# cristianpjensen/thesis-pai-reconstruction

Hardware: NVIDIA B200
Metric: pix2pix_gan_train_images_per_sec_256x256 (higher is better)
Workload: dtype bf16

## Files before the change

### include/pai_b200.h

```cpp
#ifndef PAI_B200_H
#define PAI_B200_H

#ifdef __cplusplus
extern "C" {
#endif

#define PAI_ACT_NONE 0
#define PAI_ACT_LEAKY 1
#define PAI_ACT_RELU 2
#define PAI_ACT_TANH 3

#define PAI_DTYPE_F32 0
#define PAI_DTYPE_BF16 1

const char* pai_last_error(void);
int pai_version(void);
int pai_reserve_sms(int n);

int pai_conv4x4_fprop(const void* x, int n, int h, int w, int cin, int x_ld, const void* w_packed, int cout,
                      int cout_pad, int stride, const float* bias, int act, float slope, void* y, int y_ld,
                      int y_f32, int n_tile, float* splitk_ws, void* stream);

int pai_conv4x4_fprop_dual(const void* x, int n, int h, int w, int cin, int x_ld, const void* w_packed, int cout,
                           int cout_pad, int stride, const float* bias, int act, float slope, void* y, int y_ld, void* y2,
                           int y2_ld, int act2, int n_tile, void* stream);

int pai_convT4x4s2_fprop(const void* x, int n, int h, int w, int cin, int x_ld, const void* w_packed, int cout,
                         int cout_pad, const float* bias, int act, float slope, void* y, int y_ld, int y_f32,
                         int n_tile, float* splitk_ws, void* stream);
int pai_conv4x4_fprop_bnstats(const void* x, int n, int h, int w, int cin, int x_ld, const void* w_packed, int cout,
                              int cout_pad, int stride, const float* bias, void* y, int y_ld, int n_tile,
                              float* bn_partials, int bn_rows, void* stream);
int pai_convT4x4s2_fprop_bnstats(const void* x, int n, int h, int w, int cin, int x_ld, const void* w_packed, int cout,
                                 int cout_pad, const float* bias, void* y, int y_ld, int n_tile, float* bn_partials,
                                 int bn_rows, void* stream);
int pai_conv4x4_dgrad_act(const void* gy, int n, int h, int w, int cout, int gy_ld, const void* w_packed_dgrad, int cin,
                          int cin_pad, const void* saved_act, float slope, void* gx, int gx_ld, int n_tile,
                          float* colsum_partials, int rows, void* stream);

int pai_conv4x4_wgrad(const void* x, int n, int h, int w, int cin, int x_ld, const void* gy, int cout, int gy_ld,
                      int stride, float* dw, int splitk, void* stream);
int pai_convT4x4s2_wgrad(const void* x, int n, int h, int w, int cin, int x_ld, const void* gy, int cout, int gy_ld,
                         float* dw, int splitk, void* stream);

int pai_ssim_psnr_fwd(const void* pred, const void* target, int dtype, int n, int h, int w, int denormalize,
                      float* ssim_sum, float* band_sum, float* sse, float* full_map, void* stream);
int pai_ssim_psnr_bwd(const void* pred, const void* target, int dtype, int n, int h, int w, int denormalize,
                      const float* g_ssim_sum, const float* g_sse, void* workspace, void* grad_pred, void* stream);
long long pai_ssim_bwd_workspace_bytes(int n, int h, int w);

int pai_bn_stats(const void* x, long long m, int c, int ld, float* sums, void* stream);
int pai_bn_finalize(const float* sums, long long m, int c, const float* gamma, const float* beta, float eps,
                    float momentum, int training, float* running_mean, float* running_var, float* scale_shift,
                    void* stream);
int pai_bn_finalize_partials(const float* sums, int nparts, long long m, int c, const float* gamma, const float* beta,
                             float eps, float momentum, int training, float* running_mean, float* running_var,
                             float* scale_shift, void* stream);
int pai_bn_apply_act(const void* x, long long m, int c, int ld, const float* scale_shift, void* out1, int ld1,
                     int act1, void* out2, int ld2, int act2, float slope, void* stream);
int pai_bn_bwd_reduce(const void* x, long long m, int c, int ld, const float* scale_shift, const void* g1, int ldg1,
                      int act1, const void* g2, int ldg2, int act2, float slope, float* sums, void* stream);
int pai_bn_bwd_apply(const void* x, long long m, int c, int ld, const float* scale_shift, const void* g1, int ldg1,
                     int act1, const void* g2, int ldg2, int act2, float slope, const float* sums,
                     const float* gamma, void* dx, int lddx, void* stream);
int pai_act_bwd(const void* x, long long m, int c, int ld, const void* g1, int ldg1, int act1, const void* g2, int ldg2,
                int act2, float slope, float* sums2c, void* dx, int lddx, void* stream);
// ... 129 lines not shown
```

### thesis-pai-reconstruction_b200/csrc/igemm.cu

```cuda
#include <stdio.h>
#include <stdlib.h>

#include "pai_common.cuh"
#include "pai_epilogue.cuh"
#include "pai_kernels.h"

namespace pai {

#ifdef PAI_PROFILE_ROLES
#define ROLE_T0() const long long _t0 = clock64()
#define ROLE_ADD(var) var += clock64() - _t0
#else
#define ROLE_T0()
#define ROLE_ADD(var)
#endif

static constexpr int kThreads = 256;
static constexpr int kFpropThreads = 384;
static constexpr int kMaxStages = 8;

struct __align__(8) PipeSmem {
    uint64_t full[kMaxStages];
    uint64_t empty[kMaxStages];
    uint64_t acc_full[2];
    uint64_t acc_empty[2];
    uint64_t mask_full[8];
    uint32_t tmem_base;
};

template <bool PAIR, bool MASKED>
__global__ void __launch_bounds__(kFpropThreads, 1)
igemm_fprop_kernel(const __grid_constant__ CUtensorMap tm_a, const __grid_constant__ CUtensorMap tm_b,
                   const __grid_constant__ IgemmOutMaps om, const IgemmFpropParams p) {
    pdl_launch_dependents();
    extern __shared__ uint8_t smem_raw[];
    __shared__ PipeSmem ps;
    __shared__ __align__(1024) uint4 stage_buf[8][32 * 8];
    uint8_t* smem = reinterpret_cast<uint8_t*>((reinterpret_cast<uintptr_t>(smem_raw) + 1023) & ~uintptr_t(1023));

    const int warp = threadIdx.x >> 5, lane = threadIdx.x & 31;
    const int n_tile = p.n_tile;
    const bool fused = p.fused_phases != 0;
    const uint32_t rank = PAIR ? cluster_ctarank() : 0u;
    const int cta_n = PAIR ? n_tile / 2 : n_tile;
    const uint32_t a_bytes = 128 * 128;
    const uint32_t b_bytes = (uint32_t)cta_n * 128;
    const int ksub = p.ksub;
    const uint32_t sub_bytes = a_bytes + (fused ? 4 : 1) * b_bytes;
    const uint32_t stage_bytes = (uint32_t)ksub * sub_bytes;
    const int stages = p.stages;
    const int num_kb = (fused ? 9 : p.ntaps) * p.kc_per_tap;
    const int acc_n = fused ? 4 * n_tile : n_tile;
    const uint32_t acc_cols = tmem_cols_for(acc_n);
    const int total_tiles = p.n_tiles * p.m_tiles * p.phases * p.splitk;
    const int worker = PAIR ? (int)(blockIdx.x >> 1) : (int)blockIdx.x;
    const int workers = PAIR ? (int)(gridDim.x >> 1) : (int)gridDim.x;

// ... 8 lines not shown
        }
        for (int a = 0; a < 2; ++a) {
            mbar_init(&ps.acc_full[a], 1);
            mbar_init(&ps.acc_empty[a], PAIR ? 16 : 8);
        }
        if (MASKED)
            for (int w = 0; w < 8; ++w) mbar_init(&ps.mask_full[w], 1);
        mbar_fence_init();
    }
    if (warp == 2) {
        if (PAIR)
            tmem_alloc_pair(&ps.tmem_base, 2 * acc_cols);
        else
            tmem_alloc(&ps.tmem_base, 2 * acc_cols);
    }
    tc_fence_before();
    if (PAIR)
        cluster_sync_all();
    else
        __syncthreads();
    tc_fence_after();
    const uint32_t tmem_base = ps.tmem_base;
    pdl_wait();

    long long prof_wait = 0, prof_wait2 = 0, prof_total = 0, prof_fence = 0, prof_issue = 0, prof_commit = 0;
    (void)prof_wait, (void)prof_wait2, (void)prof_total, (void)prof_fence, (void)prof_issue, (void)prof_commit;
    const int pidx = warp == 0 ? 0 : (warp == 2 ? 1 : (warp == 3 ? 2 : -1));
    if (pidx >= 0) {
        if (elect_one()) {
            constexpr int P = 3;
            int g = 0, mine = pidx;
            int stage = pidx;
            uint32_t phase = 0;
            while (stage >= stages) stage -= stages, phase ^= 1;
            const int brow = PAIR ? (int)rank * cta_n : 0;
#ifdef PAI_PROFILE_ROLES
            const long long tstart = clock64();
#endif
            for (int t = worker; t < total_tiles; t += workers) {
                int ks, tt, nt, r, mt, phase_idx, tw, th, tn;
                p.fd_splitk.divmod(t, tt, ks);
                p.fd_n_tiles.divmod(tt, r, nt);
                p.fd_m_tiles.divmod(r, phase_idx, mt);
                if (PAIR) mt = 2 * mt + (int)rank;
                p.fd_tiles_w.divmod(mt, mt, tw);
                p.fd_tiles_h.divmod(mt, tn, th);
// ... 398 lines not shown
                        } else {
#pragma unroll
                            for (int j = 0; j < 16; ++j)
                                if (col0 + cc + j < p.cout) o[j] = apply_act(f[j], p.act, p.slope);
                        }
                    } else {
                        store_bf16_16(reinterpret_cast<__nv_bfloat16*>(p.out) + off + cc, f, p.act, p.slope,
                                      vec_ok && col0 + cc + 16 <= p.cout, p.cout - (col0 + cc));
                    }
                    if (p.out2 != nullptr)
                        store_bf16_16(reinterpret_cast<__nv_bfloat16*>(p.out2) + off2 + cc, f, p.act2, p.slope,
                                      vec_ok && col0 + cc + 16 <= p.cout, p.cout - (col0 + cc));
                }
            }
            if (!released) release_acc();
#ifdef PAI_PROFILE_ROLES
            prof_total += clock64() - twork;
#endif
        }
        if (p.bn_part != nullptr) flush_stats();
        if (lane == 0) bulk_wait_group0();
#ifdef PAI_PROFILE_ROLES
        if (blockIdx.x == 0 && threadIdx.x == 128)
            printf("[roles] epilogue warp 4: waiting for a full accumulator %lld cyc, working %lld cyc over %d tiles\n", prof_wait, prof_total, it);
#endif
    }
    tc_fence_before();
    if (PAIR)
        cluster_sync_all();
    else
        __syncthreads();
    if (warp == 2) {
        tc_fence_after();
        if (PAIR)
            tmem_dealloc_pair(tmem_base, 2 * acc_cols);
        else
            tmem_dealloc(tmem_base, 2 * acc_cols);
    }
}

__global__ void __launch_bounds__(kThreads, 1)
igemm_wgrad_kernel(const __grid_constant__ CUtensorMap tm_u, const __grid_constant__ CUtensorMap tm_s,
                   const IgemmWgradParams p) {
    pdl_launch_dependents();
    extern __shared__ uint8_t smem_raw[];
    __shared__ PipeSmem ps;
    uint8_t* smem = reinterpret_cast<uint8_t*>((reinterpret_cast<uintptr_t>(smem_raw) + 1023) & ~uintptr_t(1023));

    const int warp = threadIdx.x >> 5, lane = threadIdx.x & 31;
    const int mb = p.mb, nbt = p.nbt;
    const uint32_t blk_bytes = 64 * 128;
    const uint32_t a_bytes = 2 * mb * blk_bytes;
    const uint32_t stage_bytes = a_bytes + nbt * blk_bytes;
    const int stages = p.stages;
    const int n_cols = nbt * 64;
    const uint32_t tmem_cols = tmem_cols_for(mb * 256);

    const long long units = (long long)p.tiles * p.kblocks;
    const long long u_begin = units * blockIdx.x / gridDim.x, u_end = units * (blockIdx.x + 1) / gridDim.x;

// ... 20 lines not shown
    const int pidx = warp == 0 ? 0 : (warp == 2 ? 1 : (warp == 3 ? 2 : -1));
    if (pidx >= 0) {
        if (elect_one()) {
            constexpr int P = 3;
            int stage = pidx;
            uint32_t phase = 0;
            while (stage >= stages) stage -= stages, phase ^= 1;
            for (long long u = u_begin + pidx; u < u_end; u += P) {
                const int tile = (int)(u / p.kblocks);
                int mt = (int)(u - (long long)tile * p.kblocks);
                const int ng = tile % p.n_groups, cu0 = (tile / p.n_groups) * 128 * mb;
                const int tw = mt % p.tiles_w;
                mt /= p.tiles_w;
                const int th = mt % p.tiles_h;
                const int tn = mt / p.tiles_h;
                const int w0 = tw * p.bw, h0 = th * p.bh, n0 = tn * p.bn;
                mbar_wait(&ps.empty[stage], phase ^ 1);
                uint8_t* sa = smem + (size_t)stage * stage_bytes;
                uint8_t* sb = sa + a_bytes;
                mbar_expect_tx(&ps.full[stage], stage_bytes);
                for (int i = 0; i < 2 * mb; ++i)
                    tma_load_5d(sa + i * blk_bytes, &tm_u, &ps.full[stage], cu0 + i * 64, w0, 0, h0, n0);
                for (int nb = 0; nb < nbt; ++nb) {
                    const int blk = ng * nbt + nb, tap = blk / p.cs_blocks, cb = blk - tap * p.cs_blocks;
                    tma_load_5d(sb + nb * blk_bytes, &tm_s, &ps.full[stage], p.tap_c[tap] + cb * 64, w0 + p.tap_w[tap],
                                p.tap_p[tap], h0 + p.tap_h[tap], n0);
                }
                stage += P;
                while (stage >= stages) stage -= stages, phase ^= 1;
            }
        }
    } else if (warp == 1) {
        if (elect_one()) {
            const uint32_t idesc = umma_idesc_bf16(128, n_cols, 1, 1);
            int stage = 0;
            uint32_t phase = 0;
            int seg = 0;
            long long u = u_begin;
            while (u < u_end) {
                const long long tile_end = (u / p.kblocks + 1) * p.kblocks;
                const long long seg_end = tile_end < u_end ? tile_end : u_end;
                mbar_wait(&ps.acc_empty[0], (seg & 1) ^ 1);
                tc_fence_after();
                bool first = true;
                for (; u < seg_end; ++u) {
                    mbar_wait(&ps.full[stage], phase);
                    tc_fence_after();
// ... 14 lines not shown
                        stage = 0;
                        phase ^= 1;
                    }
                }
                umma_commit(&ps.acc_full[0]);
                ++seg;
            }
        }
    } else if (warp >= 4) {
        const int q = warp & 3;
        const int r = q * 32 + lane;
        int seg = 0;
        long long u = u_begin;
        while (u < u_end) {
            const int tile = (int)(u / p.kblocks);
            const long long tile_end = (long long)(tile + 1) * p.kblocks;
            u = tile_end < u_end ? tile_end : u_end;
            const int ng = tile % p.n_groups, cu0 = (tile / p.n_groups) * 128 * mb;
            mbar_wait(&ps.acc_full[0], seg & 1);
            tc_fence_after();
            for (int a = 0; a < mb; ++a) {
                const int row = cu0 + a * 128 + r;
                const bool row_ok = row < p.cu;
                for (int nb = 0; nb < nbt; ++nb) {
                    const int blk = ng * nbt + nb, tap = blk / p.cs_blocks, cb = blk - tap * p.cs_blocks;
                    float* o = p.out + ((size_t)tap * p.cu + row) * (size_t)p.cs + cb * 64;
#pragma unroll
                    for (int c = 0; c < 64; c += 16) {
                        uint32_t v[16];
                        __syncwarp();
                        tmem_ld_16(tmem_base + ((uint32_t)(q * 32) << 16) + (uint32_t)(a * 256 + nb * 64 + c), v);
                        tmem_ld_wait();
                        if (row_ok) {
#pragma unroll
                            for (int j = 0; j < 16; j += 4)
                                red_add_v4(o + c + j, __uint_as_float(v[j]), __uint_as_float(v[j + 1]),
                                           __uint_as_float(v[j + 2]), __uint_as_float(v[j + 3]));
                        }
                    }
                }
            }
            tc_fence_before();
            __syncwarp();
            if (lane == 0) mbar_arrive_relaxed(&ps.acc_empty[0]);
            ++seg;
        }
    }
    tc_fence_before();
// ... 119 lines not shown
    if (sms < 0) return -1;
    if (blocks > sms * 8) blocks = sms * 8;
    PAI_CUDA_OK(launch_pdl(splitk_finish_kernel, dim3((unsigned)blocks), dim3(256), 0, stream, 1, ws, total, cout, bias, act, slope, y, y_ld, y_f32));
    PAI_CUDA_OK(cudaGetLastError());
    return 0;
}

int launch_igemm_wgrad(const CUtensorMap& tm_u, const CUtensorMap& tm_s, IgemmWgradParams p, cudaStream_t stream) {
    const size_t stage_bytes = (size_t)(2 * p.mb + p.nbt) * 8192;
    p.stages = pick_stages(stage_bytes, 196 * 1024);
    const size_t smem = stage_bytes * p.stages + 1024;
    static DeviceOnce once;
    const int dev = current_device(), num_sms = persistent_ctas(dev);
    if (num_sms < 0) return -1;
    if (once.need(dev)) {
        PAI_CUDA_OK(cudaFuncSetAttribute(igemm_wgrad_kernel, cudaFuncAttributeMaxDynamicSharedMemorySize, 200 * 1024));
        once.mark(dev);
    }
    const long long units = (long long)p.tiles * p.kblocks;
    long long grid = units / 4 > p.tiles ? units / 4 : p.tiles;
    if (grid > num_sms) grid = num_sms;
    if (grid < 1) grid = 1;
    if (p.max_ctas > 0 && grid > p.max_ctas) grid = p.max_ctas;
    PAI_CUDA_OK(launch_pdl(igemm_wgrad_kernel, dim3((unsigned)grid), dim3(kThreads), smem, stream, 1, tm_u, tm_s, p));
    PAI_CUDA_OK(cudaGetLastError());
    return 0;
}

}
```

### thesis-pai-reconstruction_b200/csrc/pai_api.cu

```cuda
#include <stdarg.h>
#include <stdio.h>
#include <stdlib.h>
#include <string.h>

#include <cudaTypedefs.h>

#include "pai_common.cuh"
#include "pai_kernels.h"

namespace pai {

static thread_local char g_err[512] = "";

void set_error(const char* fmt, ...) {
    va_list ap;
    va_start(ap, fmt);
    vsnprintf(g_err, sizeof(g_err), fmt, ap);
    va_end(ap);
}

int cuda_fail(cudaError_t e, const char* what) {
    set_error("CUDA error %d (%s) at %s", (int)e, cudaGetErrorString(e), what);
    return -1;
}
// ... 387 lines not shown
                         int cout_pad, const float* bias, int act, float slope, void* y, int y_ld, int y_f32,
                         int n_tile, float* splitk_ws, void* stream) {
    return convT4x4s2_fprop_impl(x, n, h, w, cin, x_ld, w_packed, cout, cout_pad, bias, act, slope, y, y_ld, y_f32, n_tile,
                                 splitk_ws, nullptr, 0, stream);
}
int pai_convT4x4s2_fprop_bnstats(const void* x, int n, int h, int w, int cin, int x_ld, const void* w_packed, int cout,
                                 int cout_pad, const float* bias, void* y, int y_ld, int n_tile, float* bn_partials,
                                 int bn_rows, void* stream) {
    PAI_REQUIRE(bn_partials != nullptr && bn_rows > 0, "pai_convT4x4s2_fprop_bnstats: null partial-sum buffer");
    return convT4x4s2_fprop_impl(x, n, h, w, cin, x_ld, w_packed, cout, cout_pad, bias, PAI_ACT_NONE, 0.f, y, y_ld, 0,
                                 n_tile, nullptr, bn_partials, bn_rows, stream);
}

int pai_conv4x4_dgrad_act(const void* gy, int n, int h, int w, int cout, int gy_ld, const void* w_packed_dgrad, int cin,
                          int cin_pad, const void* saved_act, float slope, void* gx, int gx_ld, int n_tile,
                          float* colsum_partials, int rows, void* stream) {
    PAI_REQUIRE(saved_act != nullptr, "pai_conv4x4_dgrad_act: null saved activation");
    PAI_REQUIRE(colsum_partials == nullptr || rows > 0, "pai_conv4x4_dgrad_act: bad partial-sum buffer");
    return convT4x4s2_fprop_impl(gy, n, h, w, cout, gy_ld, w_packed_dgrad, cin, cin_pad, nullptr, PAI_ACT_NONE, 0.f, gx,
                                 gx_ld, 0, n_tile, nullptr, colsum_partials, rows, stream, saved_act, slope);
}

static int wgrad_common(const void* u, int un, int uh, int uw, int cu, int u_ld, const void* s, int sh, int sw,
                        int cs, int s_ld, int stride, float* dw, int splitk, cudaStream_t stream, const char* who) {
    PAI_REQUIRE(u && s && dw, "%s: null pointer", who);
    PAI_REQUIRE(cu % 64 == 0 && cs % 64 == 0, "%s: channel counts (%d rows, %d cols) must be multiples of 64", who, cu,
                cs);
    PAI_REQUIRE(aligned16(u) && aligned16(s) && u_ld % 8 == 0 && s_ld % 8 == 0, "%s: operands must be 16 B aligned",
                who);
    PixBox b = pick_box(uw, uh, un, 64);
    CUtensorMap tm_u, tm_s;
    int rc = map_unit(&tm_u, u, un, uh, uw, cu, u_ld, b);
    if (rc) return rc;
    if (stride == 2) {
        PAI_REQUIRE(s_ld == cs && sh % 2 == 0 && sw % 2 == 0, "%s: the stride-2 operand must be dense with even h,w",
                    who);
        rc = map_split(&tm_s, s, un, sh, sw, cs, b);
    } else {
        rc = map_unit(&tm_s, s, un, sh, sw, cs, s_ld, b);
    }
    if (rc) return rc;
    IgemmWgradParams p;
    memset(&p, 0, sizeof(p));
    p.bw = b.bw, p.bh = b.bh, p.bn = b.bn, p.tiles_w = b.tiles_w, p.tiles_h = b.tiles_h, p.tiles_n = b.tiles_n;
    p.cu = cu, p.cs = cs, p.out = dw;
    for (int ky = 0; ky < 4; ++ky)
        for (int kx = 0; kx < 4; ++kx) {
            int t = ky * 4 + kx;
            if (stride == 2) {
                int qx, px, qy, py;
                s2_tap(kx, &qx, &px);
                s2_tap(ky, &qy, &py);
                p.tap_c[t] = px * cs, p.tap_w[t] = qx, p.tap_p[t] = py, p.tap_h[t] = qy;
            } else if (stride == 1) {
                p.tap_c[t] = 0, p.tap_w[t] = kx - 1, p.tap_p[t] = 0, p.tap_h[t] = ky - 1;
            }
        }
    if (stride == 3)
        for (int t = 0; t < 9; ++t) p.tap_c[t] = 0, p.tap_w[t] = t % 3 - 1, p.tap_p[t] = 0, p.tap_h[t] = t / 3 - 1;
    const int ntaps = stride == 0 ? 1 : (stride == 3 ? 9 : 16);
    p.kblocks = b.tiles_w * b.tiles_h * b.tiles_n;
    p.cs_blocks = cs / 64;
    const int nb_total = ntaps * p.cs_blocks;
    p.nbt = nb_total % 4 == 0 ? 4 : (nb_total % 2 == 0 ? 2 : 1);
    p.n_groups = nb_total / p.nbt;
    p.mb = cu > 128 ? 2 : 1;
    p.tiles = ((cu + 128 * p.mb - 1) / (128 * p.mb)) * p.n_groups;
    p.max_ctas = splitk > 0 ? splitk * p.tiles : 0;
    return launch_igemm_wgrad(tm_u, tm_s, p, stream);
}

int pai_conv4x4_wgrad(const void* x, int n, int h, int w, int cin, int x_ld, const void* gy, int cout, int gy_ld,
                      int stride, float* dw, int splitk, void* stream) {
    PAI_REQUIRE(stride == 1 || stride == 2, "pai_conv4x4_wgrad: stride must be 1 or 2");
    const int ho = stride == 2 ? h / 2 : h - 1, wo = stride == 2 ? w / 2 : w - 1;
    return wgrad_common(gy, n, ho, wo, cout, gy_ld, x, h, w, cin, x_ld, stride, dw, splitk, (cudaStream_t)stream,
                        "pai_conv4x4_wgrad");
}

int pai_pointwise_wgrad(const void* u, long long m, int cu, int u_ld, const void* s, int cs, int s_ld, float* dw,
                        int splitk, void* stream) {
    PAI_REQUIRE(m > 0 && m < (1LL << 31), "pai_pointwise_wgrad: bad row count");
    return wgrad_common(u, 1, 1, (int)m, cu, u_ld, s, 1, (int)m, cs, s_ld, 0, dw, splitk, (cudaStream_t)stream,
                        "pai_pointwise_wgrad");
}

int pai_pointwise_gemm(const void* x, long long m, int cin, int x_ld, const void* w_packed, int cout, int cout_pad,
                       const float* bias, int act, float slope, void* y, int y_ld, int y_f32, void* y2, int y2_ld,
                       int act2, int n_tile, int k_valid, void* stream) {
    PAI_REQUIRE(x && w_packed && y, "pai_pointwise_gemm: null pointer");
    PAI_REQUIRE(k_valid == 0 || (cin == 64 && k_valid > 0 && k_valid <= 64 && k_valid % 16 == 0),
                "pai_pointwise_gemm: k_valid (%d) needs cin == 64 and a multiple of 16", k_valid);
    PAI_REQUIRE(cin > 0 && cin % 64 == 0, "pai_pointwise_gemm: cin must be a multiple of 64 (got %d)", cin);
    PAI_REQUIRE(cout_pad % 16 == 0 && cout <= cout_pad, "pai_pointwise_gemm: bad cout %d / cout_pad %d", cout, cout_pad);
    PAI_REQUIRE(aligned16(x) && aligned16(w_packed) && x_ld % 8 == 0 && x_ld >= cin, "pai_pointwise_gemm: alignment");
    PAI_REQUIRE(m > 0 && m < (1LL << 31), "pai_pointwise_gemm: bad row count %lld", m);
    const int wbox = (int)m, n = 1;
    PixBox b = pick_box(wbox, 1, n, 128);
    if (n_tile <= 0) n_tile = auto_n_tile(cout_pad, (long long)b.tiles_w * b.tiles_h * b.tiles_n);
    PAI_REQUIRE(n_tile >= 16 && n_tile <= 256 && n_tile % 16 == 0 && cout_pad % n_tile == 0,
// ... 86 lines not shown
```

### thesis-pai-reconstruction_b200/csrc/pai_kernels.h

```cpp
#pragma once
#include <cuda.h>
#include <cuda_runtime.h>
#include <stdint.h>

#include "../../include/pai_b200.h"

namespace pai {

struct FastDiv {
    uint32_t mul, shift, div;
#ifdef __CUDACC__
    __device__ __forceinline__ int quot(int n) const { return (int)((__umulhi((uint32_t)n, mul) + (uint32_t)n) >> shift); }
    __device__ __forceinline__ void divmod(int n, int& q, int& r) const {
        q = quot(n);
        r = n - q * (int)div;
    }
#endif
};
inline FastDiv make_fastdiv(int d) {
    FastDiv f;
    f.div = (uint32_t)d;
    uint32_t s = 0;
    while ((1u << s) < (uint32_t)d) ++s;
    f.shift = s;
// ... 39 lines not shown
    int accumulate;
    int tma_out;
};

struct IgemmOutMaps {
    CUtensorMap out[4];
    CUtensorMap aux[4];
};

struct IgemmWgradParams {
    int bw, bh, bn;
    int tiles_w, tiles_h, tiles_n;
    int kblocks;
    int mb;
    int nbt;
    int cs_blocks;
    int n_groups;
    int tiles;
    int max_ctas;
    int cu, cs;
    int stages;
    int tap_c[16], tap_w[16], tap_p[16], tap_h[16];
    float* out;
};

bool igemm_fprop_use_pair(int n_tile, long long m_tiles, int n_tiles, int phases, int splitk);
int launch_igemm_fprop(const CUtensorMap& tm_a, const CUtensorMap& tm_b, const IgemmOutMaps& om, IgemmFpropParams p,
                       int m_tiles, int n_tiles, int phases, cudaStream_t stream);
int launch_splitk_finish(const float* ws, long long pixels, int cout, const float* bias, int act, float slope, void* y,
                         int y_ld, int y_f32, cudaStream_t stream);
int launch_igemm_wgrad(const CUtensorMap& tm_u, const CUtensorMap& tm_s, IgemmWgradParams p, cudaStream_t stream);

}
```

### thesis-pai-reconstruction_b200/pai_b200/engine.py

```python
from __future__ import annotations

import os
from typing import List, Optional

import torch

from . import dp, ops
from .ops import ACT_LEAKY, ACT_NONE, ACT_RELU, ACT_TANH

BN_EPS, BN_MOMENTUM, SLOPE = 1e-5, 0.1, 0.2
FUSE_BN_STATS = os.environ.get("PAI_NO_BN_FUSION") is None
FUSE_ACT_BWD = os.environ.get("PAI_NO_ACT_BWD_FUSION") is None
THIN_DIRECT = os.environ.get("PAI_NO_THIN_DIRECT") is None


class _PackCache:

    def get(self, tag: str, p: torch.Tensor, fn):
        store = p.__dict__.setdefault("_pai_packs", {})
        stamp = (p._version, p.data_ptr())
        ent = store.get(tag)
        if ent is None or ent[0] != stamp:
            with torch.no_grad():
                ent = (stamp, fn(p.detach()))
# ... 460 lines not shown
    if counters:
        torch._foreach_add_(counters, 1)
    if not save:
        return y, None
    s.xcol = xcol
    s.drop_masks = drop_masks
    s.plane, s.cat, s.a_in, s.raw_e, s.ss_e, s.raw_d, s.ss_d, s.dec_in0, s.y = plane, cat, a_in, raw_e, ss_e, raw_d, ss_d, dec_in0, y
    s.xc = xc
    return y, s


def unet_backward(spec: UnetSpec, s: _Saved, grad_y: torch.Tensor):
    L = spec.levels
    ch = spec.enc_ch
    y = s.y
    n, _, h, w = y.shape
    dev = y.device
    g_pre = (grad_y.float() * (1.0 - y * y)).contiguous()
    grads = {}
    last = spec.dec_convs[L - 1]
    cin_last = last.weight.shape[0]
    if spec.out_ch != 1:
        gc = _carrier(g_pre)
        dwl = ops.wgrad_finish(ops.convT4x4s2_wgrad(s.cat[L - 1], gc))
        grads[(1, L - 1)] = (dwl[:, :spec.out_ch].contiguous(), g_pre.sum((0, 2, 3)))
        dcat = ops.conv4x4_fprop(gc, _carrier_out_dgrad_pack(last.weight), cin_last, stride=2)
    else:
        g_pre = g_pre.view(n, h, w)
        gcol = None
        if THIN_DIRECT and ops.thin_wgrad_ok(s.cat[L - 1], [g_pre]):
            dw = ops.thin_conv_wgrad(s.cat[L - 1], [g_pre])
        else:
            gcol = ops.im2col4x4([g_pre], h // 2, w // 2, stride=2)
            dw = ops.pointwise_wgrad(s.cat[L - 1], gcol)
        grads[(1, L - 1)] = (dw[:, :16].reshape(cin_last, 1, 4, 4), g_pre.sum().reshape(1))
        if THIN_DIRECT and cin_last <= 256:
            dcat = _bf16(n, h // 2, w // 2, cin_last, device=dev)
            ops.thin_conv_fprop([g_pre], _thin_out_dgrad_pack(last.weight), cin_last, None, dcat, ACT_NONE)
        else:
            if gcol is None:
                gcol = ops.im2col4x4([g_pre], h // 2, w // 2, stride=2)
            dcat = ops.pointwise_gemm(gcol, _thin_out_dgrad_pack(last.weight), cin_last, k_valid=16)
    dskip = [None] * L
    for j in range(L - 2, -1, -1):
        conv, bn = spec.dec_convs[j], spec.dec_bns[j]
        co = spec.dec_out[j]
        enc_i = L - 2 - j
        dskip[enc_i] = dcat[..., co:]
        g1 = dcat[..., :co]
        raw, ss = s.raw_d[j], s.ss_d[j]
        act_out = ACT_RELU if j + 1 < L - 1 else ACT_NONE
        d_raw = _bf16(*raw.shape, device=dev)
        if ops.bn_small_ok(raw, 2):
            sums = ops.bn_small_bwd(raw, ss, g1, act_out, None, ACT_NONE, bn.weight.detach(), d_raw, slope=SLOPE,
                                    mask=s.drop_masks[j])
        else:
            if s.drop_masks[j] is not None:
                ops.scale_channels(g1, s.drop_masks[j], out=g1)
            sums = ops.bn_bwd_reduce(raw, ss, g1, act_out)
            ops.bn_bwd_apply(raw, ss, g1, act_out, None, ACT_NONE, sums, bn.weight.detach(), d_raw)
        d_in = s.cat[j] if j > 0 else s.dec_in0
        cin = conv.weight.shape[0]
        gw = ops.wgrad_finish(ops.convT4x4s2_wgrad(d_in, d_raw))
        dp.allreduce_async(gw)
        grads[(1, j)] = (gw, ops.zeros_f32(co, device=dev), sums[co:], sums[:co])
        dcat = ops.conv4x4_fprop(d_raw, _dgradT_pack(conv.weight), cin, stride=2)
    i = L - 1
    conv = spec.enc_convs[i]
    d_raw = _bf16(*s.dec_in0.shape, device=dev)
    sums = ops.act_bwd(s.dec_in0, dcat, ACT_RELU, None, ACT_NONE, d_raw)
    gw = ops.wgrad_finish(ops.conv4x4_wgrad(s.a_in[i], d_raw, stride=2))
    dp.allreduce_async(gw)
    grads[(0, i)] = (gw, sums[:ch[i]].clone())
    d_a = ops.convT4x4s2_fprop(d_raw, _dgrad_pack(conv.weight), ch[i - 1])
    for i in range(L - 2, 0, -1):
        conv, bn = spec.enc_convs[i], spec.enc_bns[i]
        raw, ss = s.raw_e[i], s.ss_e[i]
        d_raw = _bf16(*raw.shape, device=dev)
        if bn is not None and ops.bn_small_ok(raw, 3):
            sums = ops.bn_small_bwd(raw, ss, d_a, ACT_LEAKY, dskip[i], ACT_RELU, bn.weight.detach(), d_raw, slope=SLOPE)
        else:
            sums = ops.bn_bwd_reduce(raw, ss, d_a, ACT_LEAKY, dskip[i], ACT_RELU, slope=SLOPE)
            ops.bn_bwd_apply(raw, ss, d_a, ACT_LEAKY, dskip[i], ACT_RELU, sums, None if bn is None else bn.weight.detach(),
                             d_raw, slope=SLOPE)
        gw = ops.wgrad_finish(ops.conv4x4_wgrad(s.a_in[i], d_raw, stride=2))
        dp.allreduce_async(gw)
        if bn is not None:
            grads[(0, i)] = (gw, ops.zeros_f32(ch[i], device=dev), sums[ch[i]:], sums[:ch[i]])
        else:
            grads[(0, i)] = (gw, sums[:ch[i]].clone())
        d_a = ops.convT4x4s2_fprop(d_raw, _dgrad_pack(conv.weight), ch[i - 1])
    c0 = ch[0]
    d_raw = _bf16(*s.a_in[1].shape, device=dev)
    sums = ops.act_bwd(s.a_in[1], d_a, ACT_LEAKY, dskip[0], ACT_NONE, d_raw, slope=SLOPE)
    if s.xc is not None:
        dw0 = ops.wgrad_finish(ops.conv4x4_wgrad(s.xc, d_raw, stride=2))
        grads[(0, 0)] = (dw0[:, :spec.in_ch].contiguous(), sums[:c0].clone())
    else:
        if THIN_DIRECT and ops.thin_wgrad_ok(d_raw, [s.plane]):
            dw0 = ops.thin_conv_wgrad(d_raw, [s.plane])
        else:
            xcol = s.xcol if s.xcol is not None else ops.im2col4x4([s.plane], h // 2, w // 2, stride=2)
            dw0 = ops.pointwise_wgrad(d_raw, xcol)
        grads[(0, 0)] = (dw0[:, :16].reshape(c0, 1, 4, 4), sums[:c0].clone())
    out = []
    for i in range(L):
        out += list(grads[(0, i)])
    for j in range(L):
        out += list(grads[(1, j)])
    dp.finish_async()
    return out


class UnetFunction(torch.autograd.Function):
    @staticmethod
    def forward(ctx, spec: UnetSpec, training: bool, x: torch.Tensor, *params):
        need = any(ctx.needs_input_grad[3:])
        if ctx.needs_input_grad[2]:
            raise RuntimeError("pai_b200: the fused generator node has no gradient w.r.t. its input image "
# ... 88 lines not shown
    K = len(spec.convs)
    head = spec.convs[-1]
    h_last = s.hs[-1]
    c_last = h_last.shape[3]
    grads = [None] * (2 * (K - 1) + 1)
    gcol = ops.im2col4x4([g], h_last.shape[1], h_last.shape[2], stride=1, flip=True)
    if need_params:
        dwh = ops.pointwise_wgrad(h_last, gcol)[:, :16]
        grads[-1] = dwh.reshape(1, c_last, 4, 4)
    dh = ops.pointwise_gemm(gcol, _head_dgrad_pack(head.weight), c_last, k_valid=16)
    fused = None
    for k in range(K - 2, -1, -1):
        conv = spec.convs[k]
        hk = s.hs[k]
        ck = hk.shape[3]
        if fused is not None:
            d_pre, sums = fused
            fused = None
        else:
            d_pre = _bf16(*hk.shape, device=dev)
            sums = ops.act_bwd(hk, dh, ACT_LEAKY, None, ACT_NONE, d_pre, slope=SLOPE)
        if k > 0:
            if need_params:
                grads[2 * k] = ops.wgrad_finish(ops.conv4x4_wgrad(s.hs[k - 1], d_pre, stride=2))
                dp.allreduce_async(grads[2 * k])
                grads[2 * k + 1] = sums[:ck].clone()
            cprev = s.hs[k - 1].shape[3]
            if FUSE_ACT_BWD and ops.bn_fusable(s.hs[k - 1].numel() // cprev, cprev):
                d_next, part = ops.conv4x4_dgrad_act(d_pre, _dgrad_pack(conv.weight), cprev, s.hs[k - 1], slope=SLOPE,
                                                     want_colsum=need_params)
                fused = (d_next, part.sum(0) if part is not None else None)
            else:
                dh = ops.convT4x4s2_fprop(d_pre, _dgrad_pack(conv.weight), cprev)
        elif s.xyc is not None:
            h, w = s.hw
            if need_params:
                dw0 = ops.wgrad_finish(ops.conv4x4_wgrad(s.xyc, d_pre, stride=2))
                grads[0] = dw0[:, :2 * spec.img_ch].contiguous()
                grads[1] = sums[:ck].clone()
            gy = None
            if need_y:
                gyc = ops.convT4x4s2_fprop(d_pre, _carrier_in_dgrad_pack(conv.weight), CARRIER, out_f32=True)
                gy = gyc[..., spec.img_ch:2 * spec.img_ch].permute(0, 3, 1, 2).contiguous()
        else:
            h, w = s.hw
            if need_params:
                if THIN_DIRECT and ops.thin_wgrad_ok(d_pre, [s.px, s.py]):
                    dw0 = ops.thin_conv_wgrad(d_pre, [s.px, s.py])
                else:
                    xycol = s.xycol if s.xycol is not None else ops.im2col4x4([s.px, s.py], h // 2, w // 2, stride=2)
                    dw0 = ops.pointwise_wgrad(d_pre, xycol)
                grads[0] = dw0[:, :32].reshape(ck, 4, 4, 2).permute(0, 3, 1, 2)
                grads[1] = sums[:ck].clone()
            gy = None
            if need_y:
                if THIN_DIRECT and ops.thin_plane_ok(d_pre):
                    gy = ops.thin_convT_plane(d_pre, _thin_in_dgrad_pack(conv.weight, 1)).view(n, 1, h, w)
                else:
                    part = ops.pointwise_gemm(d_pre, _thin_in_dgrad_pack(conv.weight, 1), 16, out_f32=True)
                    gy = ops.col2im4x4s2(part).view(n, 1, h, w)
# ... 23 lines not shown
```

### thesis-pai-reconstruction_b200/pai_b200/lib.py

```python
from __future__ import annotations

import contextlib
import ctypes
import os

_HERE = os.path.dirname(os.path.abspath(__file__))
LIB_PATH = os.environ.get("PAI_LIB_PATH") or os.path.join(_HERE, "libpai_b200.so")

c_int, c_float, c_void_p, c_ll = ctypes.c_int, ctypes.c_float, ctypes.c_void_p, ctypes.c_longlong

SIGNATURES = {
    "pai_version": [],
    "pai_reserve_sms": [c_int],
    "pai_conv4x4_fprop": [c_void_p, c_int, c_int, c_int, c_int, c_int, c_void_p, c_int, c_int, c_int, c_void_p,
                          c_int, c_float, c_void_p, c_int, c_int, c_int, c_void_p, c_void_p],
    "pai_convT4x4s2_fprop": [c_void_p, c_int, c_int, c_int, c_int, c_int, c_void_p, c_int, c_int, c_void_p, c_int,
                             c_float, c_void_p, c_int, c_int, c_int, c_void_p, c_void_p],
    "pai_conv4x4_wgrad": [c_void_p, c_int, c_int, c_int, c_int, c_int, c_void_p, c_int, c_int, c_int, c_void_p,
                          c_int, c_void_p],
    "pai_convT4x4s2_wgrad": [c_void_p, c_int, c_int, c_int, c_int, c_int, c_void_p, c_int, c_int, c_void_p, c_int,
                             c_void_p],
    "pai_ssim_psnr_fwd": [c_void_p, c_void_p, c_int, c_int, c_int, c_int, c_int, c_void_p, c_void_p, c_void_p,
                          c_void_p, c_void_p],
    "pai_ssim_psnr_bwd": [c_void_p, c_void_p, c_int, c_int, c_int, c_int, c_int, c_void_p, c_void_p, c_void_p,
                          c_void_p, c_void_p],
    "pai_bn_stats": [c_void_p, c_ll, c_int, c_int, c_void_p, c_void_p],
    "pai_bn_finalize": [c_void_p, c_ll, c_int, c_void_p, c_void_p, c_float, c_float, c_int, c_void_p, c_void_p,
                        c_void_p, c_void_p],
    "pai_bn_apply_act": [c_void_p, c_ll, c_int, c_int, c_void_p, c_void_p, c_int, c_int, c_void_p, c_int, c_int,
                         c_float, c_void_p],
    "pai_bn_bwd_reduce": [c_void_p, c_ll, c_int, c_int, c_void_p, c_void_p, c_int, c_int, c_void_p, c_int, c_int,
                          c_float, c_void_p, c_void_p],
    "pai_bn_bwd_apply": [c_void_p, c_ll, c_int, c_int, c_void_p, c_void_p, c_int, c_int, c_void_p, c_int, c_int,
                         c_float, c_void_p, c_void_p, c_void_p, c_int, c_void_p],
    "pai_act_bwd": [c_void_p, c_ll, c_int, c_int, c_void_p, c_int, c_int, c_void_p, c_int, c_int, c_float, c_void_p,
                    c_void_p, c_int, c_void_p],
    "pai_colsum": [c_void_p, c_ll, c_int, c_int, c_void_p, c_void_p],
    "pai_bn_small_fwd": [c_void_p, c_ll, c_int, c_int, c_void_p, c_void_p, c_float, c_float, c_void_p, c_void_p, c_void_p,
                         c_void_p, c_int, c_int, c_void_p, c_int, c_int, c_float, c_void_p, c_int, c_void_p],
    "pai_bn_small_bwd": [c_void_p, c_ll, c_int, c_int, c_void_p, c_void_p, c_int, c_int, c_void_p, c_int, c_int, c_float,
                         c_void_p, c_int, c_void_p, c_void_p, c_void_p, c_int, c_void_p],
    "pai_smallc_conv_fprop": [c_void_p, c_void_p, c_int, c_int, c_int, c_int, c_int, c_int, c_int, c_int, c_void_p,
                              c_void_p, c_int, c_void_p, c_int, c_int, c_void_p, c_int, c_int, c_float, c_void_p],
    "pai_smallc_conv_wgrad": [c_void_p, c_int, c_int, c_void_p, c_void_p, c_int, c_int, c_int, c_int, c_int, c_int,
# ... 124 lines not shown
```

### thesis-pai-reconstruction_b200/pai_b200/ops.py

```python
from __future__ import annotations

import ctypes
import os

import torch

from . import lib

ACT_NONE, ACT_LEAKY, ACT_RELU, ACT_TANH = 0, 1, 2, 3
BN_SMALL_OFF = os.environ.get("PAI_NO_BN_SMALL", "0") == "1"
_T_K = ((1, 3), (0, 2))


_prof = None


def profile_start():
    global _prof
    _prof = []


def profile_stop():
    global _prof
    out, _prof = _prof, None
# ... 214 lines not shown
    ws = _splitk_ws(4 * n * h * w, cout, x.device)
    _igemm_call("pai_convT4x4s2_fprop", 2.0 * n * h * w * cout * 16 * cin, _ptr(x), n, h, w, cin, ld, _ptr(w_packed), cout, cp, _ptr(bias), act,
             float(slope), _ptr(out), old, int(out.dtype == torch.float32), n_tile, _ptr(ws), _stream())
    return out


def conv4x4_wgrad(x, gy, stride=2, dw=None, splitk=0):
    n, h, w, cin, ld = _nhwc(x)
    gn, gh, gw, cout, gld = _nhwc(gy)
    if dw is None:
        dw = torch.zeros(16, cout, cin, dtype=torch.float32, device=x.device)
    _igemm_call("pai_conv4x4_wgrad", 2.0 * gn * gh * gw * cout * 16 * cin, _ptr(x), n, h, w, cin, ld, _ptr(gy), cout, gld, stride, _ptr(dw), splitk,
             _stream())
    return dw


def convT4x4s2_wgrad(x, gy, dw=None, splitk=0):
    n, h, w, cin, ld = _nhwc(x)
    gn, gh, gw, cout, gld = _nhwc(gy)
    if dw is None:
        dw = torch.zeros(16, cin, cout, dtype=torch.float32, device=x.device)
    _igemm_call("pai_convT4x4s2_wgrad", 2.0 * n * h * w * cout * 16 * cin, _ptr(x), n, h, w, cin, ld, _ptr(gy), cout, gld, _ptr(dw), splitk, _stream())
    return dw


def dropout2d_mask(n: int, c: int, p: float, device) -> torch.Tensor:
    keep = torch.bernoulli(torch.full((n, c), 1.0 - p, dtype=torch.float32, device=device))
    return keep.mul_(1.0 / (1.0 - p))


def scale_channels(x, mask, out=None):
    n, h, w, c, ld = _nhwc(x)
    assert mask.shape == (n, c) and mask.dtype == torch.float32 and mask.is_contiguous()
    if out is None:
        out = torch.empty(n, h, w, c, dtype=torch.bfloat16, device=x.device)
    lib.call("pai_scale_channels", _ptr(x), ld, _ptr(mask), n, h * w, c, _ptr(out), _nhwc(out)[4], _stream())
    return out


def wgrad_finish(dw: torch.Tensor) -> torch.Tensor:
    _, a, b = dw.shape
    grad = torch.empty(a, b, 4, 4, dtype=torch.float32, device=dw.device)
    lib.call("pai_wgrad_finish", _ptr(dw), a * b, _ptr(grad), 0, _stream())
    return grad


# ... 560 lines not shown
```

Before: 9223.

## Write weight gradients directly in parameter layout for small-pixel wgrad layers

Adds a wgrad mode whose epilogue stores accumulators straight into the PyTorch [out,in,4,4] fp32 parameter layout. For layers with few output pixels, this replaces the zero-fill, the split-K accumulation and the separate wgrad_finish transpose. In that mode the grid is one CTA per tile with no split-K, and mb drops to 1 when enough SMs are free. This removes extra kernels and memory passes on the small bottleneck layers, but gives up split-K parallelism there. It also adds some profiling printf changes behind a compile flag.

```diff
diff --git a/include/pai_b200.h b/include/pai_b200.h
--- a/include/pai_b200.h
+++ b/include/pai_b200.h
@@ -42,6 +42,10 @@
                       int stride, float* dw, int splitk, void* stream);
 int pai_convT4x4s2_wgrad(const void* x, int n, int h, int w, int cin, int x_ld, const void* gy, int cout, int gy_ld,
                          float* dw, int splitk, void* stream);
+int pai_conv4x4_wgrad_param(const void* x, int n, int h, int w, int cin, int x_ld, const void* gy, int cout, int gy_ld,
+                            int stride, float* grad, void* stream);
+int pai_convT4x4s2_wgrad_param(const void* x, int n, int h, int w, int cin, int x_ld, const void* gy, int cout,
+                               int gy_ld, float* grad, void* stream);
 
 int pai_ssim_psnr_fwd(const void* pred, const void* target, int dtype, int n, int h, int w, int denormalize,
                       float* ssim_sum, float* band_sum, float* sse, float* full_map, void* stream);
diff --git a/thesis-pai-reconstruction_b200/csrc/igemm.cu b/thesis-pai-reconstruction_b200/csrc/igemm.cu
--- a/thesis-pai-reconstruction_b200/csrc/igemm.cu
+++ b/thesis-pai-reconstruction_b200/csrc/igemm.cu
@@ -33,6 +33,9 @@
 igemm_fprop_kernel(const __grid_constant__ CUtensorMap tm_a, const __grid_constant__ CUtensorMap tm_b,
                    const __grid_constant__ IgemmOutMaps om, const IgemmFpropParams p) {
     pdl_launch_dependents();
+#ifdef PAI_PROFILE_ROLES
+    const long long t_launch = clock64();
+#endif
     extern __shared__ uint8_t smem_raw[];
     __shared__ PipeSmem ps;
     __shared__ __align__(1024) uint4 stage_buf[8][32 * 8];
@@ -87,6 +90,9 @@
     tc_fence_after();
     const uint32_t tmem_base = ps.tmem_base;
     pdl_wait();
+#ifdef PAI_PROFILE_ROLES
+    const long long t_ready = clock64();
+#endif
 
     long long prof_wait = 0, prof_wait2 = 0, prof_total = 0, prof_fence = 0, prof_issue = 0, prof_commit = 0;
     (void)prof_wait, (void)prof_wait2, (void)prof_total, (void)prof_fence, (void)prof_issue, (void)prof_commit;
@@ -531,7 +537,9 @@
         if (lane == 0) bulk_wait_group0();
 #ifdef PAI_PROFILE_ROLES
         if (blockIdx.x == 0 && threadIdx.x == 128)
-            printf("[roles] epilogue warp 4: waiting for a full accumulator %lld cyc, working %lld cyc over %d tiles\n", prof_wait, prof_total, it);
+            printf("[roles] epilogue warp 4: prologue (launch to pdl_wait done) %lld cyc, waiting for a full accumulator %lld cyc, "
+                   "working %lld cyc over %d tiles (split-K %d), exit after %lld cyc\n",
+                   t_ready - t_launch, prof_wait, prof_total, it, p.splitk, clock64() - t_launch);
 #endif
     }
     tc_fence_before();
@@ -545,6 +553,14 @@
             tmem_dealloc_pair(tmem_base, 2 * acc_cols);
         else
             tmem_dealloc(tmem_base, 2 * acc_cols);
+    }
+}
+
+__device__ __forceinline__ void wgrad_block(const IgemmWgradParams& p, int blk, int& tap, int& cb) {
+    if (p.param_layout) {
+        tap = blk & 15, cb = blk >> 4;
+    } else {
+        tap = blk / p.cs_blocks, cb = blk - tap * p.cs_blocks;
     }
 }
 
@@ -611,7 +627,8 @@
                 for (int i = 0; i < 2 * mb; ++i)
                     tma_load_5d(sa + i * blk_bytes, &tm_u, &ps.full[stage], cu0 + i * 64, w0, 0, h0, n0);
                 for (int nb = 0; nb < nbt; ++nb) {
-                    const int blk = ng * nbt + nb, tap = blk / p.cs_blocks, cb = blk - tap * p.cs_blocks;
+                    int tap, cb;
+                    wgrad_block(p, ng * nbt + nb, tap, cb);
                     tma_load_5d(sb + nb * blk_bytes, &tm_s, &ps.full[stage], p.tap_c[tap] + cb * 64, w0 + p.tap_w[tap],
                                 p.tap_p[tap], h0 + p.tap_h[tap], n0);
                 }
@@ -672,8 +689,30 @@
             for (int a = 0; a < mb; ++a) {
                 const int row = cu0 + a * 128 + r;
                 const bool row_ok = row < p.cu;
+                if (p.param_layout) {
+                    int tap0, cb;
+                    wgrad_block(p, ng * nbt, tap0, cb);
+                    float* o = p.out + ((size_t)row * p.cs + cb * 64) * 16 + tap0;
+                    for (int c = 0; c < 64; c += 16) {
+                        uint32_t v[4][16];
+                        __syncwarp();
+#pragma unroll
+                        for (int nb = 0; nb < 4; ++nb)
+                            tmem_ld_16(tmem_base + ((uint32_t)(q * 32) << 16) + (uint32_t)(a * 256 + nb * 64 + c), v[nb]);
+                        tmem_ld_wait();
+                        if (row_ok) {
+#pragma unroll
+                            for (int j = 0; j < 16; ++j)
+                                *reinterpret_cast<float4*>(o + (size_t)(c + j) * 16) =
+                                    make_float4(__uint_as_float(v[0][j]), __uint_as_float(v[1][j]),
+                                                __uint_as_float(v[2][j]), __uint_as_float(v[3][j]));
+                        }
+                    }
+                    continue;
+                }
                 for (int nb = 0; nb < nbt; ++nb) {
-                    const int blk = ng * nbt + nb, tap = blk / p.cs_blocks, cb = blk - tap * p.cs_blocks;
+                    int tap, cb;
+                    wgrad_block(p, ng * nbt + nb, tap, cb);
                     float* o = p.out + ((size_t)tap * p.cu + row) * (size_t)p.cs + cb * 64;
 #pragma unroll
                     for (int c = 0; c < 64; c += 16) {
@@ -839,6 +878,7 @@
     if (grid > num_sms) grid = num_sms;
     if (grid < 1) grid = 1;
     if (p.max_ctas > 0 && grid > p.max_ctas) grid = p.max_ctas;
+    if (p.param_layout) grid = p.tiles;
     PAI_CUDA_OK(launch_pdl(igemm_wgrad_kernel, dim3((unsigned)grid), dim3(kThreads), smem, stream, 1, tm_u, tm_s, p));
     PAI_CUDA_OK(cudaGetLastError());
     return 0;
diff --git a/thesis-pai-reconstruction_b200/csrc/pai_api.cu b/thesis-pai-reconstruction_b200/csrc/pai_api.cu
--- a/thesis-pai-reconstruction_b200/csrc/pai_api.cu
+++ b/thesis-pai-reconstruction_b200/csrc/pai_api.cu
@@ -433,7 +433,8 @@
 }
 
 static int wgrad_common(const void* u, int un, int uh, int uw, int cu, int u_ld, const void* s, int sh, int sw,
-                        int cs, int s_ld, int stride, float* dw, int splitk, cudaStream_t stream, const char* who) {
+                        int cs, int s_ld, int stride, float* dw, int splitk, cudaStream_t stream, const char* who,
+                        bool param_layout = false) {
     PAI_REQUIRE(u && s && dw, "%s: null pointer", who);
     PAI_REQUIRE(cu % 64 == 0 && cs % 64 == 0, "%s: channel counts (%d rows, %d cols) must be multiples of 64", who, cu,
                 cs);
@@ -476,6 +477,12 @@
     p.nbt = nb_total % 4 == 0 ? 4 : (nb_total % 2 == 0 ? 2 : 1);
     p.n_groups = nb_total / p.nbt;
     p.mb = cu > 128 ? 2 : 1;
+    if (param_layout) {
+        const int sms = sm_count(current_device());
+        if (sms < 0) return -1;
+        p.param_layout = 1;
+        if (((cu + 127) / 128) * p.n_groups <= sms) p.mb = 1;
+    }
     p.tiles = ((cu + 128 * p.mb - 1) / (128 * p.mb)) * p.n_groups;
     p.max_ctas = splitk > 0 ? splitk * p.tiles : 0;
     return launch_igemm_wgrad(tm_u, tm_s, p, stream);
@@ -487,6 +494,20 @@
     const int ho = stride == 2 ? h / 2 : h - 1, wo = stride == 2 ? w / 2 : w - 1;
     return wgrad_common(gy, n, ho, wo, cout, gy_ld, x, h, w, cin, x_ld, stride, dw, splitk, (cudaStream_t)stream,
                         "pai_conv4x4_wgrad");
+}
+
+int pai_conv4x4_wgrad_param(const void* x, int n, int h, int w, int cin, int x_ld, const void* gy, int cout, int gy_ld,
+                            int stride, float* grad, void* stream) {
+    PAI_REQUIRE(stride == 1 || stride == 2, "pai_conv4x4_wgrad_param: stride must be 1 or 2");
+    const int ho = stride == 2 ? h / 2 : h - 1, wo = stride == 2 ? w / 2 : w - 1;
+    return wgrad_common(gy, n, ho, wo, cout, gy_ld, x, h, w, cin, x_ld, stride, grad, 0, (cudaStream_t)stream,
+                        "pai_conv4x4_wgrad_param", true);
+}
+
+int pai_convT4x4s2_wgrad_param(const void* x, int n, int h, int w, int cin, int x_ld, const void* gy, int cout,
+                               int gy_ld, float* grad, void* stream) {
+    return wgrad_common(x, n, h, w, cin, x_ld, gy, 2 * h, 2 * w, cout, gy_ld, 2, grad, 0, (cudaStream_t)stream,
+                        "pai_convT4x4s2_wgrad_param", true);
 }
 
 int pai_pointwise_wgrad(const void* u, long long m, int cu, int u_ld, const void* s, int cs, int s_ld, float* dw,
diff --git a/thesis-pai-reconstruction_b200/csrc/pai_kernels.h b/thesis-pai-reconstruction_b200/csrc/pai_kernels.h
--- a/thesis-pai-reconstruction_b200/csrc/pai_kernels.h
+++ b/thesis-pai-reconstruction_b200/csrc/pai_kernels.h
@@ -85,6 +85,7 @@
     int stages;
     int tap_c[16], tap_w[16], tap_p[16], tap_h[16];
     float* out;
+    int param_layout;
 };
 
 bool igemm_fprop_use_pair(int n_tile, long long m_tiles, int n_tiles, int phases, int splitk);
diff --git a/thesis-pai-reconstruction_b200/pai_b200/engine.py b/thesis-pai-reconstruction_b200/pai_b200/engine.py
--- a/thesis-pai-reconstruction_b200/pai_b200/engine.py
+++ b/thesis-pai-reconstruction_b200/pai_b200/engine.py
@@ -506,7 +506,7 @@
     cin_last = last.weight.shape[0]
     if spec.out_ch != 1:
         gc = _carrier(g_pre)
-        dwl = ops.wgrad_finish(ops.convT4x4s2_wgrad(s.cat[L - 1], gc))
+        dwl = ops.convT4x4s2_weight_grad(s.cat[L - 1], gc)
         grads[(1, L - 1)] = (dwl[:, :spec.out_ch].contiguous(), g_pre.sum((0, 2, 3)))
         dcat = ops.conv4x4_fprop(gc, _carrier_out_dgrad_pack(last.weight), cin_last, stride=2)
     else:
@@ -545,7 +545,7 @@
             ops.bn_bwd_apply(raw, ss, g1, act_out, None, ACT_NONE, sums, bn.weight.detach(), d_raw)
         d_in = s.cat[j] if j > 0 else s.dec_in0
         cin = conv.weight.shape[0]
-        gw = ops.wgrad_finish(ops.convT4x4s2_wgrad(d_in, d_raw))
+        gw = ops.convT4x4s2_weight_grad(d_in, d_raw)
         dp.allreduce_async(gw)
         grads[(1, j)] = (gw, ops.zeros_f32(co, device=dev), sums[co:], sums[:co])
         dcat = ops.conv4x4_fprop(d_raw, _dgradT_pack(conv.weight), cin, stride=2)
@@ -553,7 +553,7 @@
     conv = spec.enc_convs[i]
     d_raw = _bf16(*s.dec_in0.shape, device=dev)
     sums = ops.act_bwd(s.dec_in0, dcat, ACT_RELU, None, ACT_NONE, d_raw)
-    gw = ops.wgrad_finish(ops.conv4x4_wgrad(s.a_in[i], d_raw, stride=2))
+    gw = ops.conv4x4_weight_grad(s.a_in[i], d_raw, stride=2)
     dp.allreduce_async(gw)
     grads[(0, i)] = (gw, sums[:ch[i]].clone())
     d_a = ops.convT4x4s2_fprop(d_raw, _dgrad_pack(conv.weight), ch[i - 1])
@@ -567,7 +567,7 @@
             sums = ops.bn_bwd_reduce(raw, ss, d_a, ACT_LEAKY, dskip[i], ACT_RELU, slope=SLOPE)
             ops.bn_bwd_apply(raw, ss, d_a, ACT_LEAKY, dskip[i], ACT_RELU, sums, None if bn is None else bn.weight.detach(),
                              d_raw, slope=SLOPE)
-        gw = ops.wgrad_finish(ops.conv4x4_wgrad(s.a_in[i], d_raw, stride=2))
+        gw = ops.conv4x4_weight_grad(s.a_in[i], d_raw, stride=2)
         dp.allreduce_async(gw)
         if bn is not None:
             grads[(0, i)] = (gw, ops.zeros_f32(ch[i], device=dev), sums[ch[i]:], sums[:ch[i]])
@@ -578,7 +578,7 @@
     d_raw = _bf16(*s.a_in[1].shape, device=dev)
     sums = ops.act_bwd(s.a_in[1], d_a, ACT_LEAKY, dskip[0], ACT_NONE, d_raw, slope=SLOPE)
     if s.xc is not None:
-        dw0 = ops.wgrad_finish(ops.conv4x4_wgrad(s.xc, d_raw, stride=2))
+        dw0 = ops.conv4x4_weight_grad(s.xc, d_raw, stride=2)
         grads[(0, 0)] = (dw0[:, :spec.in_ch].contiguous(), sums[:c0].clone())
     else:
         if THIN_DIRECT and ops.thin_wgrad_ok(d_raw, [s.plane]):
@@ -713,7 +713,7 @@
             sums = ops.act_bwd(hk, dh, ACT_LEAKY, None, ACT_NONE, d_pre, slope=SLOPE)
         if k > 0:
             if need_params:
-                grads[2 * k] = ops.wgrad_finish(ops.conv4x4_wgrad(s.hs[k - 1], d_pre, stride=2))
+                grads[2 * k] = ops.conv4x4_weight_grad(s.hs[k - 1], d_pre, stride=2)
                 dp.allreduce_async(grads[2 * k])
                 grads[2 * k + 1] = sums[:ck].clone()
             cprev = s.hs[k - 1].shape[3]
@@ -726,7 +726,7 @@
         elif s.xyc is not None:
             h, w = s.hw
             if need_params:
-                dw0 = ops.wgrad_finish(ops.conv4x4_wgrad(s.xyc, d_pre, stride=2))
+                dw0 = ops.conv4x4_weight_grad(s.xyc, d_pre, stride=2)
                 grads[0] = dw0[:, :2 * spec.img_ch].contiguous()
                 grads[1] = sums[:ck].clone()
             gy = None
diff --git a/thesis-pai-reconstruction_b200/pai_b200/lib.py b/thesis-pai-reconstruction_b200/pai_b200/lib.py
--- a/thesis-pai-reconstruction_b200/pai_b200/lib.py
+++ b/thesis-pai-reconstruction_b200/pai_b200/lib.py
@@ -20,6 +20,10 @@
                           c_int, c_void_p],
     "pai_convT4x4s2_wgrad": [c_void_p, c_int, c_int, c_int, c_int, c_int, c_void_p, c_int, c_int, c_void_p, c_int,
                              c_void_p],
+    "pai_conv4x4_wgrad_param": [c_void_p, c_int, c_int, c_int, c_int, c_int, c_void_p, c_int, c_int, c_int, c_void_p,
+                                c_void_p],
+    "pai_convT4x4s2_wgrad_param": [c_void_p, c_int, c_int, c_int, c_int, c_int, c_void_p, c_int, c_int, c_void_p,
+                                   c_void_p],
     "pai_ssim_psnr_fwd": [c_void_p, c_void_p, c_int, c_int, c_int, c_int, c_int, c_void_p, c_void_p, c_void_p,
                           c_void_p, c_void_p],
     "pai_ssim_psnr_bwd": [c_void_p, c_void_p, c_int, c_int, c_int, c_int, c_int, c_void_p, c_void_p, c_void_p,
diff --git a/thesis-pai-reconstruction_b200/pai_b200/ops.py b/thesis-pai-reconstruction_b200/pai_b200/ops.py
--- a/thesis-pai-reconstruction_b200/pai_b200/ops.py
+++ b/thesis-pai-reconstruction_b200/pai_b200/ops.py
@@ -260,6 +260,35 @@
         dw = torch.zeros(16, cin, cout, dtype=torch.float32, device=x.device)
     _igemm_call("pai_convT4x4s2_wgrad", 2.0 * n * h * w * cout * 16 * cin, _ptr(x), n, h, w, cin, ld, _ptr(gy), cout, gld, _ptr(dw), splitk, _stream())
     return dw
+
+
+WGRAD_PARAM_MAX_PIXELS = 16 * 64
+
+
+def conv4x4_weight_grad(x, gy, stride=2, param_layout=None):
+    n, h, w, cin, ld = _nhwc(x)
+    gn, gh, gw, cout, gld = _nhwc(gy)
+    if param_layout is None:
+        param_layout = gn * gh * gw <= WGRAD_PARAM_MAX_PIXELS
+    if not param_layout:
+        return wgrad_finish(conv4x4_wgrad(x, gy, stride=stride))
+    grad = torch.empty(cout, cin, 4, 4, dtype=torch.float32, device=x.device)
+    _igemm_call("pai_conv4x4_wgrad_param", 2.0 * gn * gh * gw * cout * 16 * cin, _ptr(x), n, h, w, cin, ld, _ptr(gy), cout,
+                gld, stride, _ptr(grad), _stream())
+    return grad
+
+
+def convT4x4s2_weight_grad(x, gy, param_layout=None):
+    n, h, w, cin, ld = _nhwc(x)
+    gn, gh, gw, cout, gld = _nhwc(gy)
+    if param_layout is None:
+        param_layout = n * h * w <= WGRAD_PARAM_MAX_PIXELS
+    if not param_layout:
+        return wgrad_finish(convT4x4s2_wgrad(x, gy))
+    grad = torch.empty(cin, cout, 4, 4, dtype=torch.float32, device=x.device)
+    _igemm_call("pai_convT4x4s2_wgrad_param", 2.0 * n * h * w * cout * 16 * cin, _ptr(x), n, h, w, cin, ld, _ptr(gy), cout,
+                gld, _ptr(grad), _stream())
+    return grad
 
 
 def dropout2d_mask(n: int, c: int, p: float, device) -> torch.Tensor:
```

Result: faster. 9330, median of 6 (+1.2%).
